# cryscan/bevy-hikari

Measured on AMD Instinct MI355X. Metric: Mray/s (Cornell 1080p 2-bounce, whole job) + frame ms, higher is better.
Workload: dtype f32

## Files before the change

### bevy-hikari_amd/csrc/kernels_denoise.hip

```cpp
#include <hip/hip_runtime.h>

#include "hk_device.hpp"
#include "hk_kernels.hpp"

#ifndef HK_DENOISE_W
#define HK_DENOISE_W 64
#endif
static_assert(HK_DENOISE_W == 64, "pixel_known_empty (hk_kernels.hpp) takes a wave for one row of pixels");

namespace hkd {

__global__ __launch_bounds__(256) void k_derive_planes(GBuffer g, float* __restrict__ depth_plane, float4* __restrict__ dn_g, int width, int row_begin,
                                                       int row_end) {
  const Pixel px = pixel_of_thread(width, row_begin, row_end);
  if (!px.valid) return;
  const int idx = px.x + width * px.y;
  const float depth = g.position[idx].w;
  depth_plane[idx] = depth;
  dn_g[idx] = denoise_geometry(g.normal[idx], g.instance_material[idx].x);
}

__global__ __launch_bounds__(256) void k_count_geometry_rows(const float* __restrict__ depth, int width, uint32_t* __restrict__ out) {
  __shared__ uint32_t partial[4];
  const int y = (int)blockIdx.x;
  uint32_t n = 0;
  for (int x = (int)threadIdx.x; x < width; x += 256) n += !(depth[(size_t)y * width + x] < HK_F32_EPSILON) ? 1u : 0u;
  for (int off = 32; off > 0; off >>= 1) n += __shfl_down(n, off);
  if ((threadIdx.x & 63) == 0) partial[threadIdx.x >> 6] = n;
  __syncthreads();
  if (threadIdx.x == 0) out[y] = partial[0] + partial[1] + partial[2] + partial[3];
}

template <int NCH>
__global__ __launch_bounds__(256) void k_demodulation(DFrame fr, DemodTargets d, int row_begin, int row_end) {
  const Pixel px = pixel_of_thread_rows<64, true>(fr.rw, row_begin, row_end);
  if (!px.valid) return;
  const int x = px.x, y = px.y, index = x + fr.rw * y;
  const int tile_bits = d.empty_tiles ? pixel_tile_bits(d.empty_tiles, d.tiles_x, x, y, 1, fr.rw, fr.rh) : 0;
  if (__ballot(tile_bits == 0) == 0ull) {
    if (__ballot(tile_bits < HK_TILE_POST_KEPT) == 0ull) return;
    const uint32_t at8 = (uint32_t)index * 8u, at4 = (uint32_t)index * 4u;
#pragma unroll
    for (int ch = 0; ch < NCH; ++ch) {
      *reinterpret_cast<uint2*>(reinterpret_cast<char*>(d.output[ch]) + at8) = make_uint2(0u, 0x3C000000u);
      *reinterpret_cast<float*>(reinterpret_cast<char*>(d.internal_variance[ch]) + at4) = 0.0f;
    }
    return;
  }
  const f2 uv = coords_to_uv(fr, x, y);
  const f2 deferred_uv = jittered_deferred_uv(fr, uv, 0.5f);
  int ax, ay, rx, ry;
  nearest_coords(deferred_uv, fr.dw, fr.dh, &ax, &ay);
  const f3 albedo = xyz(unpack_f16x4(d.albedo[ax + fr.dw * ay]));
  nearest_coords(uv, fr.rw, fr.rh, &rx, &ry);
  uint2 render_in[NCH];
#pragma unroll
  for (int ch = 0; ch < NCH; ++ch) render_in[ch] = d.render[ch][rx + fr.rw * ry];
  float tap_variance[9][NCH];
  bool tap_inside[9];
#pragma unroll
  for (int ox = -1; ox <= 1; ++ox) {
#pragma unroll
    for (int oy = -1; oy <= 1; ++oy) {
      const int k = (ox + 1) * 3 + (oy + 1);
      const f2 sample_uv = uv + F2((float)ox * fr.inv_rw, (float)oy * fr.inv_rh);
      tap_inside[k] = !(sample_uv.x < 0.0f || sample_uv.y < 0.0f || sample_uv.x > 1.0f || sample_uv.y > 1.0f);
      int sx, sy;
      nearest_coords(sample_uv, fr.rw, fr.rh, &sx, &sy);
      const int at = tap_inside[k] ? sx + fr.rw * sy : index;
#pragma unroll
      for (int ch = 0; ch < NCH; ++ch) tap_variance[k][ch] = d.variance[ch][at];
    }
  }
#pragma unroll
  for (int ch = 0; ch < NCH; ++ch) {
    f3 irradiance = xyz(unpack_f16x4(render_in[ch]));
    const f3 qd = irradiance / albedo;
    irradiance = F3(albedo.x < 0.01f ? 0.0f : qd.x, albedo.y < 0.01f ? 0.0f : qd.y, albedo.z < 0.01f ? 0.0f : qd.z);
    d.output[ch][index] = pack_f16x4(F4(irradiance, 1.0f));
  }
  float sum_variance[NCH];
#pragma unroll
  for (int ch = 0; ch < NCH; ++ch) sum_variance[ch] = 0.0f;
#pragma unroll
  for (int ox = -1; ox <= 1; ++ox) {
#pragma unroll
    for (int oy = -1; oy <= 1; ++oy) {
      const int k = (ox + 1) * 3 + (oy + 1);
#pragma unroll
      for (int ch = 0; ch < NCH; ++ch) {
        const float variance = tap_variance[k][ch];
        const float with_tap = sum_variance[ch] + fr.kernel[(oy + 1) * 3 + (ox + 1)] * fmax_(variance, 0.0f);
        sum_variance[ch] = (tap_inside[k] && !(variance > HK_F32_MAX)) ? with_tap : sum_variance[ch];
      }
    }
  }
#pragma unroll
  for (int ch = 0; ch < NCH; ++ch) d.internal_variance[ch][index] = sum_variance[ch];
}

__device__ __forceinline__ bool nan_or_above_max(f3 v) { return !(v.x <= HK_F32_MAX) || !(v.y <= HK_F32_MAX) || !(v.z <= HK_F32_MAX); }

#ifndef HK_DENOISE_WAVES
#define HK_DENOISE_WAVES 8
#endif
template <int LEVEL, int NCH, int FFMASK>
__global__ __launch_bounds__(256, HK_DENOISE_WAVES) void k_denoise(DFrame fr, DenoiseTargets d, int row_begin, int row_end) {
  const Pixel px = pixel_of_thread_rows<HK_DENOISE_W, false>(fr.rw, row_begin, row_end);
  if (!px.valid) return;
  constexpr int STEP = 8 >> LEVEL;
  const int x = px.x, y = px.y, index = x + fr.rw * y;
  const int tile_bits = d.empty_tiles ? pixel_tile_bits(d.empty_tiles, d.tiles_x, x, y, 0, fr.rw, fr.rh) : 0;
  if (__ballot(tile_bits == 0) == 0ull) {
    if (__ballot(tile_bits < HK_TILE_POST_KEPT) != 0ull) {
#pragma unroll
      for (int ch = 0; ch < NCH; ++ch) d.output[ch][index] = make_uint2(0u, 0u);
    }
    if (LEVEL == 3 && d.tone_mapped && !(d.tone_kept && __ballot(tile_bits != (HK_TILE_EMPTY | HK_TILE_KEPT | HK_TILE_POST_KEPT)) == 0ull))
      d.tone_mapped[index] = pack_f16x4(F4(d.clear_color[0], d.clear_color[1], d.clear_color[2], d.clear_color[3]));
    return;
  }
  int col_texel[3], row_texel[3];
  bool col_inside[3], row_inside[3];
#pragma unroll
  for (int a = 0; a < 3; ++a) {
    const f2 tap_uv = coords_to_uv(fr, x + (a - 1) * STEP, y + (a - 1) * STEP);
    col_inside[a] = !(tap_uv.x < 0.0f || tap_uv.x > 1.0f);
    row_inside[a] = !(tap_uv.y < 0.0f || tap_uv.y > 1.0f);
    nearest_coords(jittered_deferred_uv(fr, tap_uv, 0.5f), fr.dw, fr.dh, &col_texel[a], &row_texel[a]);
  }
  const int dx = col_texel[1], dy = row_texel[1];
  const int didx = dx + fr.dw * dy;
  const float4 gc = d.dn_g[didx];
  const float depth = d.depth[didx];
  if (depth < HK_F32_EPSILON) {
#pragma unroll
    for (int ch = 0; ch < NCH; ++ch) d.output[ch][index] = make_uint2(0u, 0u);
    if (LEVEL == 3 && d.tone_mapped) d.tone_mapped[index] = pack_f16x4(F4(d.clear_color[0], d.clear_color[1], d.clear_color[2], d.clear_color[3]));
    return;
  }
  const float2 dg = d.depth_gradient[didx];
  const f2 depth_gradient = F2(dg.x, dg.y);
  const f3 normal = F3(gc.x, gc.y, gc.z);
  const float instance = gc.w;

  constexpr int OX[8] = {-1, 0, 1, -1, 1, -1, 0, 1};
  constexpr int OY[8] = {-1, -1, -1, 0, 0, 1, 1, 1};
  bool tap_inside[8];
  float w_geometry[8];
#pragma unroll
  for (int k = 0; k < 8; ++k) {
    const int ox = OX[k], oy = OY[k];
    tap_inside[k] = col_inside[ox + 1] && row_inside[oy + 1];
    w_geometry[k] = 0.0f;
    if (tap_inside[k]) {
      const int gx = col_texel[ox + 1], gy = row_texel[oy + 1];
      const float4 gs = d.dn_g[gx + fr.dw * gy];
      const float sample_depth = d.depth[gx + fr.dw * gy];
      const f3 sample_normal = F3(gs.x, gs.y, gs.z);
      const float w_normal = pow16_(fmax_(0.0f, dot(normal, sample_normal)));
      const float w_depth = exp_nonpositive_((-fabsf(depth - sample_depth)) / (fabsf(dot(depth_gradient, F2((float)ox, (float)oy))) + 0.01f));
      const float w_instance = fmax_(0.0f, 1.0f - fabsf(instance - gs.w));
      w_geometry[k] = w_normal * w_depth * w_instance;
    }
  }
  f4 albedo = F4(0, 0, 0, 0), tone_sum = F4(0, 0, 0, 0);
  if (LEVEL == 3) albedo = unpack_f16x4(d.albedo[didx]);
#pragma unroll
  for (int ch = 0; ch < NCH; ++ch) {
    const float variance = d.internal_variance[ch][index];
    const uint2 centre = d.input[ch][index];
    f3 irradiance = xyz(unpack_f16x4(centre));
    f3 sum_irradiance = irradiance * fr.kernel[4];
    float sum_w = fr.kernel[4];
    if (nan_or_above_max(irradiance)) {
      irradiance = F3(0, 0, 0);
      sum_irradiance = F3(0, 0, 0);
      sum_w = 0.0f;
    }
    const float lum = luminance(irradiance);
    const float lum_denominator = 4.0f * pow_quarter_(variance) + 0.001f;
    const double inv_lum_denominator = 1.0 / (double)lum_denominator;
    uint2 tap[8];
#pragma unroll
    for (int k = 0; k < 8; ++k) tap[k] = tap_inside[k] ? d.input[ch][index + OX[k] * STEP + fr.rw * (OY[k] * STEP)] : make_uint2(0u, 0u);
    float ff_moment_1 = 0.0f, ff_moment_2 = 0.0f, ff_count = 0.0f;
    bool black = (centre.x | (centre.y & 0xFFFFu)) == 0u && lum_denominator == lum_denominator;
#pragma unroll
    for (int k = 0; k < 8; ++k) black = black && (tap[k].x | (tap[k].y & 0xFFFFu)) == 0u;
    if (__ballot(!black) == 0ull) {
#pragma unroll
      for (int k = 0; k < 8; ++k) {
        if (!tap_inside[k]) continue;
        const float w = clamp_(w_geometry[k] * 1.0f, 0.0f, 1.0f) * fr.kernel[(OY[k] + 1) * 3 + (OX[k] + 1)];
        const float zw = 0.0f * w;
        sum_irradiance = sum_irradiance + F3(zw, zw, zw);
        sum_w += w;
      }
    } else {
#pragma unroll
      for (int k = 0; k < 8; ++k) {
        if (!tap_inside[k]) continue;
        const f3 irr = xyz(unpack_f16x4(tap[k]));
        if (nan_or_above_max(irr)) continue;
        const float sample_luminance = luminance(irr);
        const float w_luminance = exp_nonpositive_(quotient_by_reciprocal(-fabsf(lum - sample_luminance), inv_lum_denominator));
        const float w = clamp_(w_geometry[k] * w_luminance, 0.0f, 1.0f) * fr.kernel[(OY[k] + 1) * 3 + (OX[k] + 1)];
        sum_irradiance = sum_irradiance + irr * w;
        sum_w += w;
        if ((FFMASK >> ch) & 1) {
          ff_moment_1 += sample_luminance;
          ff_moment_2 += sample_luminance * sample_luminance;
          ff_count += 1.0f;
        }
      }
    }
    const f3 qd = sum_irradiance / sum_w;
    irradiance = (sum_w < 0.0001f) ? F3(0, 0, 0) : qd;
    if ((FFMASK >> ch) & 1) {
      const float ff_mean = ff_moment_1 / ff_count;
      const float ff_var = ff_moment_2 / ff_count - ff_mean * ff_mean;
      if (lum > ff_mean + 3.0f * sqrtf(ff_var)) irradiance = ff_mean / lum * irradiance;
    }
    f4 color = F4(irradiance, 1.0f);
    if (LEVEL == 3) color = color * albedo;
    const uint2 packed = pack_f16x4(color);
    d.output[ch][index] = packed;
    if (LEVEL == 3) tone_sum = (ch == 0) ? unpack_f16x4(packed) : tone_sum + unpack_f16x4(packed);
  }
  if (LEVEL == 3 && d.tone_mapped) {
    const f3 c = F3(fmax_(tone_sum.x, 0.0039f), fmax_(tone_sum.y, 0.0039f), fmax_(tone_sum.z, 0.0039f));
    const float l_old = dot(c, F3(0.2126f, 0.7152f, 0.0722f));
    const float l_new = l_old / (1.0f + l_old);
    f4 o = F4(c * (l_new / l_old), tone_sum.w);
    if (!(tone_sum.w > 0.0f)) o = F4(d.clear_color[0], d.clear_color[1], d.clear_color[2], d.clear_color[3]);
    d.tone_mapped[index] = pack_f16x4(o);
  }
}

}

namespace hk {
using namespace hkd;

void launch_derive_planes(hipStream_t st, const GBuffer& g, float* depth_plane, void* dn_g, int width, int y0, int y1) {
  if (y1 <= y0) return;
  hipLaunchKernelGGL(k_derive_planes, grid_for(width, y1 - y0), dim3(256), 0, st, g, depth_plane, (float4*)dn_g, width, y0, y1);
}

void launch_count_geometry_rows(hipStream_t st, const float* depth, int width, int height, uint32_t* out) {
  if (height <= 0) return;
  hipLaunchKernelGGL(k_count_geometry_rows, dim3((unsigned)height), dim3(256), 0, st, depth, width, out);
}

void launch_demodulation(hipStream_t st, int nch, const DFrame& fr, const DemodTargets& d, int y0, int y1) {
  if (y1 <= y0) return;
  dim3 grid = grid_for_rows(64, fr.rw, y1 - y0);
  switch (nch) {
    case 1: hipLaunchKernelGGL(k_demodulation<1>, grid, dim3(256), 0, st, fr, d, y0, y1); break;
    case 2: hipLaunchKernelGGL(k_demodulation<2>, grid, dim3(256), 0, st, fr, d, y0, y1); break;
    default: hipLaunchKernelGGL(k_demodulation<3>, grid, dim3(256), 0, st, fr, d, y0, y1); break;
  }
}

template <int LEVEL>
static void launch_denoise_level(hipStream_t st, int nch, int ffmask, const DFrame& fr, const DenoiseTargets& d, int y0, int y1) {
  dim3 grid = grid_for_rows(HK_DENOISE_W, fr.rw, y1 - y0);
  if (nch == 1 && ffmask == 0) hipLaunchKernelGGL((k_denoise<LEVEL, 1, 0>), grid, dim3(256), 0, st, fr, d, y0, y1);
  else if (nch == 1) hipLaunchKernelGGL((k_denoise<LEVEL, 1, 1>), grid, dim3(256), 0, st, fr, d, y0, y1);
  else if (nch == 2) hipLaunchKernelGGL((k_denoise<LEVEL, 2, 2>), grid, dim3(256), 0, st, fr, d, y0, y1);
  else hipLaunchKernelGGL((k_denoise<LEVEL, 3, 6>), grid, dim3(256), 0, st, fr, d, y0, y1);
}
void launch_denoise(hipStream_t st, int level, int nch, int ffmask, const DFrame& fr, const DenoiseTargets& d, int y0, int y1) {
  if (y1 <= y0) return;
  switch (level) {
    case 0: launch_denoise_level<0>(st, nch, ffmask, fr, d, y0, y1); break;
    case 1: launch_denoise_level<1>(st, nch, ffmask, fr, d, y0, y1); break;
    case 2: launch_denoise_level<2>(st, nch, ffmask, fr, d, y0, y1); break;
    default: launch_denoise_level<3>(st, nch, ffmask, fr, d, y0, y1); break;
  }
}

}
```

Measured before the change: 7813.

## Batch and hoist denoise gather loads with branch-free addressing and sched barriers

Restructures the denoise kernel's memory access. Geometry taps are loaded in batches of four, with out-of-bounds taps clamped to the centre texel, so the loads can issue together before the weight math runs. Per-channel input taps are loaded unconditionally using byte offsets, the depth-gradient load is hoisted above the early exit, and a branch-free exp replaces the previous helper. Scheduling barriers and asm register pins enforce the ordering. This trades extra (redundant) loads and register pressure for more memory-level parallelism.

```diff
diff --git a/bevy-hikari_amd/csrc/kernels_denoise.hip b/bevy-hikari_amd/csrc/kernels_denoise.hip
--- a/bevy-hikari_amd/csrc/kernels_denoise.hip
+++ b/bevy-hikari_amd/csrc/kernels_denoise.hip
@@ -103,6 +103,38 @@
 
 #ifndef HK_DENOISE_WAVES
 #define HK_DENOISE_WAVES 8
+#endif
+__device__ __forceinline__ float exp_nonpositive_flat_(float x) {
+  const bool is_nan = x != x, underflows = x < -103.972084045410f;
+  const float a = (is_nan || underflows) ? 0.0f : x;
+  const float z = floorf(fmaf(1.44269504088896341f, a, 0.5f));
+  float r = fmaf(z, -0.693359375f, a);
+  r = fmaf(z, 2.12194440e-4f, r);
+  float p = fmaf(1.9875691500e-4f, r, 1.3981999507e-3f);
+  p = fmaf(p, r, 8.3334519073e-3f);
+  p = fmaf(p, r, 4.1665795894e-2f);
+  p = fmaf(p, r, 1.6666665459e-1f);
+  p = fmaf(p, r, 5.0000001201e-1f);
+  const float y = scale2(fmaf(p, r * r, r) + 1.0f, (int)z);
+  return is_nan ? x : underflows ? 0.0f : y;
+}
+
+template <class T>
+__device__ __forceinline__ T load_at_byte(const T* plane, uint32_t byte) {
+  return *reinterpret_cast<const T*>(reinterpret_cast<const char*>(plane) + byte);
+}
+template <class T>
+__device__ __forceinline__ T load_texel(const T* plane, int texel) {
+  return load_at_byte(plane, (uint32_t)texel * (uint32_t)sizeof(T));
+}
+
+struct ChannelTexels {
+  float variance;
+  uint2 centre, tap[8];
+};
+
+#ifndef HK_DENOISE_TAP_BATCH
+#define HK_DENOISE_TAP_BATCH 4
 #endif
 template <int LEVEL, int NCH, int FFMASK>
 __global__ __launch_bounds__(256, HK_DENOISE_WAVES) void k_denoise(DFrame fr, DenoiseTargets d, int row_begin, int row_end) {
@@ -133,13 +165,14 @@
   const int didx = dx + fr.dw * dy;
   const float4 gc = d.dn_g[didx];
   const float depth = d.depth[didx];
+  const float2 dg = d.depth_gradient[didx];
+  __builtin_amdgcn_sched_barrier(0);
   if (depth < HK_F32_EPSILON) {
 #pragma unroll
     for (int ch = 0; ch < NCH; ++ch) d.output[ch][index] = make_uint2(0u, 0u);
     if (LEVEL == 3 && d.tone_mapped) d.tone_mapped[index] = pack_f16x4(F4(d.clear_color[0], d.clear_color[1], d.clear_color[2], d.clear_color[3]));
     return;
   }
-  const float2 dg = d.depth_gradient[didx];
   const f2 depth_gradient = F2(dg.x, dg.y);
   const f3 normal = F3(gc.x, gc.y, gc.z);
   const float instance = gc.w;
@@ -149,27 +182,59 @@
   bool tap_inside[8];
   float w_geometry[8];
 #pragma unroll
-  for (int k = 0; k < 8; ++k) {
-    const int ox = OX[k], oy = OY[k];
-    tap_inside[k] = col_inside[ox + 1] && row_inside[oy + 1];
-    w_geometry[k] = 0.0f;
-    if (tap_inside[k]) {
-      const int gx = col_texel[ox + 1], gy = row_texel[oy + 1];
-      const float4 gs = d.dn_g[gx + fr.dw * gy];
-      const float sample_depth = d.depth[gx + fr.dw * gy];
-      const f3 sample_normal = F3(gs.x, gs.y, gs.z);
+  for (int k = 0; k < 8; ++k) tap_inside[k] = col_inside[OX[k] + 1] && row_inside[OY[k] + 1];
+#pragma unroll
+  for (int b = 0; b < 8; b += HK_DENOISE_TAP_BATCH) {
+    float4 gs[HK_DENOISE_TAP_BATCH];
+    float sample_depth[HK_DENOISE_TAP_BATCH];
+#pragma unroll
+    for (int j = 0; j < HK_DENOISE_TAP_BATCH; ++j) {
+      const int k = b + j;
+      if (k >= 8) break;
+      const int at = tap_inside[k] ? col_texel[OX[k] + 1] + fr.dw * row_texel[OY[k] + 1] : didx;
+      gs[j] = load_texel(d.dn_g, at);
+      sample_depth[j] = load_texel(d.depth, at);
+    }
+    __builtin_amdgcn_sched_barrier(0);
+#pragma unroll
+    for (int j = 0; j < HK_DENOISE_TAP_BATCH; ++j) {
+      const int k = b + j;
+      if (k >= 8) break;
+      const int ox = OX[k], oy = OY[k];
+      const f3 sample_normal = F3(gs[j].x, gs[j].y, gs[j].z);
       const float w_normal = pow16_(fmax_(0.0f, dot(normal, sample_normal)));
-      const float w_depth = exp_nonpositive_((-fabsf(depth - sample_depth)) / (fabsf(dot(depth_gradient, F2((float)ox, (float)oy))) + 0.01f));
-      const float w_instance = fmax_(0.0f, 1.0f - fabsf(instance - gs.w));
-      w_geometry[k] = w_normal * w_depth * w_instance;
-    }
-  }
-  f4 albedo = F4(0, 0, 0, 0), tone_sum = F4(0, 0, 0, 0);
-  if (LEVEL == 3) albedo = unpack_f16x4(d.albedo[didx]);
+      const float w_depth = exp_nonpositive_flat_((-fabsf(depth - sample_depth[j])) / (fabsf(dot(depth_gradient, F2((float)ox, (float)oy))) + 0.01f));
+      const float w_instance = fmax_(0.0f, 1.0f - fabsf(instance - gs[j].w));
+      const float w = w_normal * w_depth * w_instance;
+      w_geometry[k] = tap_inside[k] ? w : 0.0f;
+      asm volatile("" : "+v"(w_geometry[k]));
+    }
+    __builtin_amdgcn_sched_barrier(0);
+  }
+  f4 tone_sum = F4(0, 0, 0, 0);
+  uint2 albedo_packed = make_uint2(0u, 0u);
+  if (LEVEL == 3) albedo_packed = d.albedo[didx];
+  ChannelTexels texels[NCH];
+  auto load_channel = [&](int ch) {
+    int own_byte = index * 8;
+    asm volatile("" : "+v"(own_byte));
+    texels[ch].variance = load_texel(d.internal_variance[ch], index);
+    texels[ch].centre = load_at_byte(d.input[ch], (uint32_t)own_byte);
+    int row_byte[3];
+#pragma unroll
+    for (int b = 0; b < 3; ++b) row_byte[b] = row_inside[b] ? own_byte + fr.rw * ((b - 1) * STEP * 8) : own_byte;
+#pragma unroll
+    for (int k = 0; k < 8; ++k) {
+      const int in_row = row_byte[OY[k] + 1];
+      texels[ch].tap[k] = load_at_byte(d.input[ch], (uint32_t)(col_inside[OX[k] + 1] ? in_row + OX[k] * STEP * 8 : in_row));
+    }
+  };
 #pragma unroll
   for (int ch = 0; ch < NCH; ++ch) {
-    const float variance = d.internal_variance[ch][index];
-    const uint2 centre = d.input[ch][index];
+    load_channel(ch);
+    __builtin_amdgcn_sched_barrier(0);
+    const float variance = texels[ch].variance;
+    const uint2 centre = texels[ch].centre;
     f3 irradiance = xyz(unpack_f16x4(centre));
     f3 sum_irradiance = irradiance * fr.kernel[4];
     float sum_w = fr.kernel[4];
@@ -183,7 +248,7 @@
     const double inv_lum_denominator = 1.0 / (double)lum_denominator;
     uint2 tap[8];
 #pragma unroll
-    for (int k = 0; k < 8; ++k) tap[k] = tap_inside[k] ? d.input[ch][index + OX[k] * STEP + fr.rw * (OY[k] * STEP)] : make_uint2(0u, 0u);
+    for (int k = 0; k < 8; ++k) tap[k] = tap_inside[k] ? texels[ch].tap[k] : make_uint2(0u, 0u);
     float ff_moment_1 = 0.0f, ff_moment_2 = 0.0f, ff_count = 0.0f;
     bool black = (centre.x | (centre.y & 0xFFFFu)) == 0u && lum_denominator == lum_denominator;
 #pragma unroll
@@ -223,7 +288,10 @@
       if (lum > ff_mean + 3.0f * sqrtf(ff_var)) irradiance = ff_mean / lum * irradiance;
     }
     f4 color = F4(irradiance, 1.0f);
-    if (LEVEL == 3) color = color * albedo;
+    if (LEVEL == 3) {
+      asm volatile("" : "+v"(albedo_packed.x), "+v"(albedo_packed.y));
+      color = color * unpack_f16x4(albedo_packed);
+    }
     const uint2 packed = pack_f16x4(color);
     d.output[ch][index] = packed;
     if (LEVEL == 3) tone_sum = (ch == 0) ? unpack_f16x4(packed) : tone_sum + unpack_f16x4(packed);
```

After: 7919, median of 4. 1.4% higher.
